# awslabs/dgl-ke

Measured on NVIDIA H100. Metric: edges/sec TransE_l2 d=400 neg=200 at 1/2/4/8 H100 vs ref CPU; HBM GB/s %peak, higher is better.
Workload: dtype f32

## Files before the change

### dgl-ke_b200/csrc/kge_rows.cu

```cuda
#include "kge_common.cuh"

namespace kge {


constexpr int kRowBlock = 256;
constexpr int kWarpsPerBlock = kRowBlock / kWarp;

__global__ void __launch_bounds__(kRowBlock) k_gather(TableView t, const long long* __restrict__ idx,
                                                       long long n, float* __restrict__ out) {
  long long job = (long long)blockIdx.x * kWarpsPerBlock + (threadIdx.x >> 5);
  if (job >= n) return;
  int lane = threadIdx.x & 31;
  const float* src = row_ptr(t, idx[job]);
  float* dst = out + job * (long long)t.dim;
  int nv = t.dim >> 2;
  for (int v = lane; v < nv; v += kWarp) st4(dst + 4 * v, ld4_stream(src + 4 * v));
  for (int k = (nv << 2) + lane; k < t.dim; k += kWarp) dst[k] = src[k];
}

void launch_gather(const LaunchCtx& c, const TableView& t, const long long* idx, long long n, float* out) {
  if (n <= 0) return;
  KGE_LAUNCH(c, k_gather, ceil_div(n, kWarpsPerBlock), kRowBlock, 0, t, idx, n, out);
}

// ... 458 lines not shown
  if (lane == 0) {
    float ps = pos[i];
    float wb = wt ? *wbar : 1.f;
    if (p.pairwise) {
      pl[i] = 0.f;
      gpos[i] = gp;
    } else {
      float dd;
      pl[i] = crit(r, ps, 1.f, dd);
      gpos[i] = dd * wb * r.inv2B;
    }
    nl[i] = nls;
    if (r.l2) rowsum[i] = rs;
  }
}

__global__ void __launch_bounds__(256) k_colsum(StepParams p, const float* __restrict__ V, float* __restrict__ colsum) {
  __shared__ float part[8][33];
  const int c = blockIdx.y, j = blockIdx.x * 32 + (threadIdx.x & 31), w = threadIdx.x >> 5;
  float s = 0.f;
  if (j < p.Ns) {
    const float* v = V + ((long long)c * p.Cs) * p.Ns + j;
    for (int i = w; i < p.Cs; i += 8) s += v[(long long)i * p.Ns];
  }
  part[w][threadIdx.x & 31] = s;
  __syncthreads();
  if (w == 0 && j < p.Ns) {
    float t = 0.f;
#pragma unroll
    for (int q = 0; q < 8; ++q) t += part[q][threadIdx.x];
    colsum[(long long)c * p.Ns + j] = t;
  }
}

__device__ __forceinline__ float block_sum(float v, float* sh) {
  v = warp_sum(v);
  int w = threadIdx.x >> 5, l = threadIdx.x & 31;
  __syncthreads();
  if (l == 0) sh[w] = v;
  __syncthreads();
  float r = (threadIdx.x < (blockDim.x >> 5)) ? sh[threadIdx.x] : 0.f;
  if (w == 0) r = warp_sum(r);
  return r;
}

__global__ void __launch_bounds__(1024) k_mean(const float* __restrict__ x, long long n, float* __restrict__ out) {
  __shared__ float sh[32];
  float s = 0.f;
  for (long long i = threadIdx.x; i < n; i += blockDim.x) s += x[i];
  s = block_sum(s, sh);
  if (threadIdx.x == 0) *out = s / (float)n;
}

constexpr int kRedBlocks = 64;
__device__ void reduce_log_part(const StepParams& p, const StepWs& w, long long nreg, const float* wbar, float* log4,
                                int bid, int nb) {
  __shared__ float sh[32];
  __shared__ bool last;
  const float *pl = w.pl, *nl = w.nl, *regp = w.regp;
  float* partial = w.red_partial;
  unsigned int* ticket = w.red_ticket;
  float a = 0.f, b = 0.f, r = 0.f;
  const long long t0 = (long long)bid * blockDim.x + threadIdx.x, stride = (long long)nb * blockDim.x;
  for (long long i = t0; i < p.B; i += stride) { a += pl[i]; b += nl[i]; }
  for (long long i = t0; i < nreg; i += stride) r += regp[i];
  a = block_sum(a, sh);
  b = block_sum(b, sh);
  r = block_sum(r, sh);
  if (threadIdx.x == 0) {
    partial[bid * 3 + 0] = a; partial[bid * 3 + 1] = b; partial[bid * 3 + 2] = r;
    __threadfence();
    unsigned int t = atomicAdd(ticket, 1u);
    last = (t == (unsigned int)nb - 1);
  }
  __syncthreads();
  if (last) {
    __threadfence();
    float sa = 0.f, sb = 0.f, sr = 0.f;
    if ((int)threadIdx.x < nb) {
      sa = ((volatile float*)partial)[threadIdx.x * 3 + 0];
      sb = ((volatile float*)partial)[threadIdx.x * 3 + 1];
      sr = ((volatile float*)partial)[threadIdx.x * 3 + 2];
    }
    sa = block_sum(sa, sh);
    sb = block_sum(sb, sh);
    sr = block_sum(sr, sh);
    if (threadIdx.x == 0) {
      float pos_loss = sa / (float)p.B * (wbar ? *wbar : 1.f);
      float neg_loss = sb / (float)p.B;
      log4[0] = p.pairwise ? 0.f : pos_loss; log4[1] = p.pairwise ? 0.f : neg_loss;
      log4[2] = p.pairwise ? neg_loss : (neg_loss + pos_loss) / 2.f;
      log4[3] = p.reg_coef * sr;
      *ticket = 0u;
    }
  }
}

__global__ void __launch_bounds__(256) k_reduce_log(StepParams p, StepWs w, long long nreg, const float* __restrict__ wbar,
                                                     float* __restrict__ log4) {
  if (nreg > 0 && p.U_dev) nreg = p.B + p.Nn + *p.U_dev;
  reduce_log_part(p, w, nreg, wbar, log4, blockIdx.x, gridDim.x);
}

void launch_wbar(const LaunchCtx& c, const StepParams& p, const float* wt, const StepWs& w) {
  if (wt) KGE_LAUNCH(c, k_mean, 1, 1024, 0, wt, p.B, w.wbar);
}

void launch_reduce_log(const LaunchCtx& c, const StepParams& p, const float* wt, const StepWs& w, float* log4,
                       bool want_reg) {
  const bool reg_on = want_reg && (p.reg_coef > 0.f && p.reg_norm > 0);
  if (log4)
    KGE_LAUNCH(c, k_reduce_log, kRedBlocks, 256, 0, p, w, reg_on ? (p.B + p.Nn + p.U) : 0, wt ? w.wbar : nullptr, log4);
}

void launch_loss_rows(const LaunchCtx& c, const StepParams& p, const float* pos, const float* S, const float* wt,
                      const StepWs& w) {
  KGE_LAUNCH(c, k_loss, ceil_div(p.B, kWarpsPerBlock), kRowBlock, 0, p, pos, S, wt, w.wbar, w.V, w.gpos, w.rowsum,
             w.pl, w.nl, w.Vhi, w.Vlo, w.VhiT, w.VloT);
}

void launch_colsum(const LaunchCtx& c, const StepParams& p, const StepWs& w) {
  if (p.model == KGE_TRANSE_L2) KGE_LAUNCH(c, k_colsum, dim3(ceil_div(p.Ns, 32), p.C), 256, 0, p, w.V, w.colsum);
}

void launch_loss(const LaunchCtx& c, const StepParams& p, const float* pos, const float* S, const float* wt,
                 const StepWs& w, float* log4, bool want_reg) {
  launch_wbar(c, p, wt, w);
  launch_loss_rows(c, p, pos, S, wt, w);
  launch_colsum(c, p, w);
  launch_reduce_log(c, p, wt, w, log4, want_reg);
}

template <int MODEL, int KIT>
__global__ void __launch_bounds__(kRowBlock) k_chain(StepParams p, TableView ent, TableView rel, BatchView b, StepWs w) {
  const long long i = (long long)blockIdx.x * kWarpsPerBlock + (threadIdx.x >> 5);
  if (i >= p.B) return;
  const int lane = threadIdx.x & 31;
  const long long hl = b.head_local[i], tl = b.tail_local[i], rid = b.rel_ids[i];
  const float* h = head_row(p, ent, b, w, i);
  const float* t = tail_row(p, ent, b, w, i);
  const float* r = row_ptr(rel, rid);
  const float* ga = w.GA + i * (long long)p.D;
  float* ngh = w.NG + hl * (long long)p.D;
  float* ngt = w.NG + tl * (long long)p.D;
  float* gr = p.rel_dense ? (w.rg + rid * (long long)p.Dr) : (w.GR + i * (long long)p.Dr);
  const bool dense = p.rel_dense != 0;
  auto rel_out = [&](int col, float4 v) { if (dense) red_add4(gr + col, v); else st4(gr + col, v); };
  const float gp = w.gpos[i];
  float gs = 0.f;

  if (MODEL == KGE_COMPLEX || MODEL == KGE_ROTATE) {
    const int half = p.D >> 1, nvh = half >> 2;
    const float den = p.emb_init / 3.14159265358979323846f;
    for (int v = lane; v < nvh; v += kWarp) {
      float4 hr = ld4(h + 4 * v), hi = ld4(h + half + 4 * v);
      float4 tr = ld4(t + 4 * v), ti = ld4(t + half + 4 * v);
      float4 gre = ld4(ga + 4 * v), gim = ld4(ga + half + 4 * v);
      float4 cr, ci, ph;
      if (MODEL == KGE_COMPLEX) { cr = ld4(r + 4 * v); ci = ld4(r + half + 4 * v); }
      else { ph = ld4(r + 4 * v); phase_cos_sin(ph, den, cr, ci); }
      float4 dhr, dhi, dtr, dti, dcr, dci;
      if (MODEL == KGE_COMPLEX) {
        dhr = f4_scale(f4_add(f4_mul(tr, cr), f4_mul(ti, ci)), gp);
        dhi = f4_scale(f4_sub(f4_mul(ti, cr), f4_mul(tr, ci)), gp);
        dtr = f4_scale(f4_sub(f4_mul(hr, cr), f4_mul(hi, ci)), gp);
        dti = f4_scale(f4_add(f4_mul(hi, cr), f4_mul(hr, ci)), gp);
        dcr = f4_scale(f4_add(f4_mul(hr, tr), f4_mul(hi, ti)), gp);
        dci = f4_scale(f4_sub(f4_mul(hr, ti), f4_mul(hi, tr)), gp);
      } else {
        float4 dre = f4_sub(f4_sub(f4_mul(hr, cr), f4_mul(hi, ci)), tr);
        float4 dim = f4_sub(f4_add(f4_mul(hr, ci), f4_mul(hi, cr)), ti);
        float4 qre, qim;
#define KGE_Q(c_)                                                                    \
        { float m = sqrtf(dre.c_ * dre.c_ + dim.c_ * dim.c_); float s_ = (m > 0.f) ? (-gp / m) : 0.f; \
          qre.c_ = dre.c_ * s_; qim.c_ = dim.c_ * s_; }
        KGE_Q(x) KGE_Q(y) KGE_Q(z) KGE_Q(w)
#undef KGE_Q
        dhr = f4_add(f4_mul(qre, cr), f4_mul(qim, ci));
        dhi = f4_sub(f4_mul(qim, cr), f4_mul(qre, ci));
        dtr = f4_neg(qre);
        dti = f4_neg(qim);
        dcr = f4_add(f4_mul(qre, hr), f4_mul(qim, hi));
        dci = f4_sub(f4_mul(qim, hr), f4_mul(qre, hi));
      }
      if (p.neg_head) {
        dtr = f4_add(dtr, f4_sub(f4_mul(gre, cr), f4_mul(gim, ci)));
        dti = f4_add(dti, f4_add(f4_mul(gre, ci), f4_mul(gim, cr)));
        dcr = f4_add(dcr, f4_add(f4_mul(gre, tr), f4_mul(gim, ti)));
        dci = f4_add(dci, f4_sub(f4_mul(gre, ti), f4_mul(gim, tr)));
      } else {
        dhr = f4_add(dhr, f4_add(f4_mul(gre, cr), f4_mul(gim, ci)));
        dhi = f4_add(dhi, f4_sub(f4_mul(gim, cr), f4_mul(gre, ci)));
        dcr = f4_add(dcr, f4_add(f4_mul(gre, hr), f4_mul(gim, hi)));
        dci = f4_add(dci, f4_sub(f4_mul(gim, hr), f4_mul(gre, hi)));
      }
      red_add4(ngh + 4 * v, dhr); red_add4(ngh + half + 4 * v, dhi);
      red_add4(ngt + 4 * v, dtr); red_add4(ngt + half + 4 * v, dti);
      if (MODEL == KGE_COMPLEX) {
        float4 g0 = f4_add(dcr, reg_grad4(cr, p.reg_norm, p.reg_coef));
        float4 g1 = f4_add(dci, reg_grad4(ci, p.reg_norm, p.reg_coef));
        rel_out(4 * v, g0); rel_out(half + 4 * v, g1);
        gs += f4_dot(g0, g0) + f4_dot(g1, g1);
      } else {
        float4 dth = f4_sub(f4_mul(dci, cr), f4_mul(dcr, ci));
        float4 g0 = make_float4(dth.x / den, dth.y / den, dth.z / den, dth.w / den);
        g0 = f4_add(g0, reg_grad4(ph, p.reg_norm, p.reg_coef));
        rel_out(4 * v, g0);
        gs += f4_dot(g0, g0);
      }
    }
  } else {
    const int nv = p.D >> 2;
    float nrm_scale = 0.f, rsum = 0.f;
    if (MODEL == KGE_TRANSE_L2) {
      float n = w.pnorm[i];
      nrm_scale = (n > 0.f) ? (-gp / n) : 0.f;
      rsum = w.rowsum[i];
    }
    const float4 z4 = make_float4(0.f, 0.f, 0.f, 0.f);
    for (int v0 = 0; v0 < nv; v0 += kWarp * KIT) {
      float4 hq[KIT], rq[KIT], tq[KIT], gq[KIT];
#pragma unroll
      for (int it = 0; it < KIT; ++it) {
        const int v = v0 + lane + kWarp * it;
        const bool ok = v < nv;
        hq[it] = ok ? ld4(h + 4 * v) : z4; rq[it] = ok ? ld4(r + 4 * v) : z4;
        tq[it] = ok ? ld4(t + 4 * v) : z4; gq[it] = ok ? ld4(ga + 4 * v) : z4;
      }
#pragma unroll
      for (int it = 0; it < KIT; ++it) {
        const int v = v0 + lane + kWarp * it;
        if (v >= nv) continue;
        const float4 h4 = hq[it], r4 = rq[it], t4 = tq[it], g4 = gq[it];
        float4 dh, dt, dr;
        if (MODEL == KGE_TRANSE_L1 || MODEL == KGE_TRANSE_L2) {
          float4 e = f4_sub(f4_add(h4, r4), t4);
          float4 u;
          if (MODEL == KGE_TRANSE_L2) u = f4_scale(e, nrm_scale);
          else u = make_float4(-gp * sgnf(e.x), -gp * sgnf(e.y), -gp * sgnf(e.z), -gp * sgnf(e.w));
          float4 a = p.neg_head ? f4_sub(t4, r4) : f4_add(h4, r4);
          float4 gA = (MODEL == KGE_TRANSE_L2) ? f4_fma(a, -rsum, g4) : g4;
          if (p.neg_head) { dt = f4_sub(gA, u); dr = f4_sub(u, gA); dh = u; }
          else            { dh = f4_add(u, gA); dr = dh; dt = f4_neg(u); }
        } else {
          dh = f4_scale(f4_mul(r4, t4), gp);
          dr = f4_scale(f4_mul(h4, t4), gp);
          dt = f4_scale(f4_mul(h4, r4), gp);
          if (p.neg_head) { dt = f4_add(dt, f4_mul(g4, r4)); dr = f4_add(dr, f4_mul(g4, t4)); }
          else            { dh = f4_add(dh, f4_mul(g4, r4)); dr = f4_add(dr, f4_mul(g4, h4)); }
        }
        red_add4(ngh + 4 * v, dh);
        red_add4(ngt + 4 * v, dt);
        dr = f4_add(dr, reg_grad4(r4, p.reg_norm, p.reg_coef));
        rel_out(4 * v, dr);
        gs += f4_dot(dr, dr);
      }
    }
  }
  gs = warp_sum(gs);
  if (lane == 0) {
    if (dense) atomicAdd(w.rgs + rid, gs / (float)p.Dr);
    else w.gsr[i] = gs / (float)p.Dr;
  }
}

void launch_chain(const LaunchCtx& c, const StepParams& p, const TableView& ent, const TableView& rel,
                  const BatchView& b, const StepWs& w) {
  if (ent.n_shards > 1) {
    KGE_DISPATCH_MODEL(p.model, KGE_LAUNCH(c, (k_chain<M, 4>), ceil_div(p.B, kWarpsPerBlock), kRowBlock, 0, p, ent, rel, b, w));
  } else {
    KGE_DISPATCH_MODEL(p.model, KGE_LAUNCH(c, (k_chain<M, 1>), ceil_div(p.B, kWarpsPerBlock), kRowBlock, 0, p, ent, rel, b, w));
  }
}

struct UpdArgs {
  StepParams p;
  TableView ent, rel;
  BatchView b;
  StepWs w;
  float* log4;
  const float* wt;
  int phase_lo, phase_hi;
  int bulk_red;
};

__device__ __forceinline__ unsigned int ld_acquire_u32(const unsigned int* p) {
  unsigned int v;
  asm volatile("ld.acquire.gpu.global.u32 %0, [%1];" : "=r"(v) : "l"(p) : "memory");
  return v;
}
__device__ __forceinline__ void grid_barrier(unsigned int* ctr) {
  __syncthreads();
  if (threadIdx.x == 0) {
    __threadfence();
    atomicAdd(ctr, 1u);
    while (ld_acquire_u32(ctr) < gridDim.x) __nanosleep(200);
    __threadfence();
  }
  __syncthreads();
}

constexpr int kRedRowFloats = 512;
struct RedStage {
  float* buf[2];
  unsigned n;
};
__device__ __forceinline__ float* red_stage_acquire(RedStage& r, int lane) {
  if (lane == 0) asm volatile("cp.async.bulk.wait_group.read 1;" ::: "memory");
  __syncwarp();
  return r.buf[r.n & 1u];
}
__device__ __forceinline__ void red_stage_issue(RedStage& r, float* dst, int dim, int lane) {
  asm volatile("fence.proxy.async.shared::cta;" ::: "memory");
  __syncwarp();
  if (lane == 0) {
    asm volatile("cp.reduce.async.bulk.global.shared::cta.bulk_group.add.f32 [%0], [%1], %2;"
                 :: "l"(dst), "r"((unsigned)__cvta_generic_to_shared(r.buf[r.n & 1u])), "r"((unsigned)dim * 4u) : "memory");
    asm volatile("cp.async.bulk.commit_group;" ::: "memory");
  }
  ++r.n;
}
__device__ __forceinline__ void red_stage_drain(int lane) {
  if (lane == 0) asm volatile("cp.async.bulk.wait_group 0;" ::: "memory");
  __syncwarp();
}
__device__ __forceinline__ void st_shared4(float* p, float4 v) { *reinterpret_cast<float4*>(p) = v; }

__device__ __forceinline__ void upd_node(const StepParams& p, const TableView& ent, const BatchView& b, const StepWs& w,
                                         long long u, int lane, RedStage* rs) {
  const long long id = b.node_ids[u];
  float* row = row_ptr(ent, id);
  float* ng = w.NG + u * (long long)p.D;
  const float* nc = node_row(p, ent, b, w, u);
  const int nv = p.D >> 2;
  const float4 z = make_float4(0.f, 0.f, 0.f, 0.f);
  const bool sharded = ent.n_shards > 1;
  const bool reg_on = (p.reg_coef > 0.f && p.reg_norm > 0);
  float* st = state_ptr(ent, id);
  if (nv <= 4 * kWarp) {
    float4 x[4], gq[4];
#pragma unroll
    for (int q = 0; q < 4; ++q) {
      const int v = lane + kWarp * q;
      x[q] = (v < nv) ? ld4(nc + 4 * v) : z;
      gq[q] = (v < nv) ? ld4(ng + 4 * v) : z;
    }
    float gs = 0.f, reg = 0.f;
#pragma unroll
    for (int q = 0; q < 4; ++q) {
      gq[q] = f4_add(gq[q], reg_grad4(x[q], p.reg_norm, p.reg_coef));
      gs += f4_dot(gq[q], gq[q]);
      if (reg_on && node_reg_in_update(p)) reg += abs_pow4_sum(x[q], p.reg_norm);
    }
    gs = warp_sum(gs) / (float)p.D;
    if (node_reg_in_update(p)) {
      reg = warp_sum(reg);
      if (lane == 0) w.regp[p.B + p.Nn + u] = reg;
    }
    float* st = state_ptr(ent, id);
    float s_new = 0.f;
    if (lane == 0) {
      if (sharded) s_new = atomicAdd_system(st, gs) + gs;
      else { s_new = *st + gs; *st = s_new; }
    }
    s_new = __shfl_sync(0xffffffffu, s_new, 0);
    const float nlr_std = -p.lr / (sqrtf(s_new) + 1e-10f);
    float* stage = (sharded && rs) ? red_stage_acquire(*rs, lane) : nullptr;
#pragma unroll
    for (int q = 0; q < 4; ++q) {
      const int v = lane + kWarp * q;
      if (v < nv) {
        if (stage) st_shared4(stage + 4 * v, f4_scale(gq[q], nlr_std));
        else if (sharded) red_add4_sys(row + 4 * v, f4_scale(gq[q], nlr_std));
        else st4(row + 4 * v, f4_fma(gq[q], nlr_std, x[q]));
        st4(ng + 4 * v, z);
      }
    }
    if (stage) red_stage_issue(*rs, row, p.D, lane);
    return;
  }
  float gs = 0.f, reg = 0.f;
  for (int v = lane; v < nv; v += kWarp) {
    const float4 x = ld4(nc + 4 * v);
    float4 g = f4_add(ld4(ng + 4 * v), reg_grad4(x, p.reg_norm, p.reg_coef));
    gs += f4_dot(g, g);
    if (reg_on && node_reg_in_update(p)) reg += abs_pow4_sum(x, p.reg_norm);
  }
  gs = warp_sum(gs) / (float)p.D;
  if (node_reg_in_update(p)) {
    reg = warp_sum(reg);
    if (lane == 0) w.regp[p.B + p.Nn + u] = reg;
  }
  float s_new = 0.f;
  if (lane == 0) {
    if (sharded) s_new = atomicAdd_system(st, gs) + gs;
    else { s_new = *st + gs; *st = s_new; }
  }
  s_new = __shfl_sync(0xffffffffu, s_new, 0);
  const float stdv = sqrtf(s_new) + 1e-10f;
  const float nlr_std = -p.lr / stdv;
  for (int v = lane; v < nv; v += kWarp) {
    float4 x = ld4(nc + 4 * v);
    float4 g = f4_add(ld4(ng + 4 * v), reg_grad4(x, p.reg_norm, p.reg_coef));
    const float4 tmp = f4_scale(g, nlr_std);
    if (sharded) red_add4_sys(row + 4 * v, tmp);
    else st4(row + 4 * v, f4_add(x, tmp));
    st4(ng + 4 * v, z);
  }
}

__device__ __forceinline__ void upd_rel_dense(const TableView& rel, float* rg, float* rgs, long long r, float lr, int lane) {
  const float gs = rgs[r];
  if (gs == 0.f) return;
  float* st = state_ptr(rel, r);
  float s_new = 0.f;
  if (lane == 0) { s_new = *st + gs; *st = s_new; }
  s_new = __shfl_sync(0xffffffffu, s_new, 0);
  __syncwarp();
  if (lane == 0) rgs[r] = 0.f;
  const float stdv = sqrtf(s_new) + 1e-10f;
  float* row = row_ptr(rel, r);
  float* g = rg + r * (long long)rel.dim;
  const float4 z = make_float4(0.f, 0.f, 0.f, 0.f);
  for (int v = lane; v < (rel.dim >> 2); v += kWarp) {
    float4 x = ld4(g + 4 * v), e = ld4(row + 4 * v);
    st4(row + 4 * v, f4_fma(x, -lr / stdv, e));
    st4(g + 4 * v, z);
  }
}

__device__ __forceinline__ void apply_row(const TableView& t, long long id, const float* g, int dim, float lr, int lane,
                                          RedStage* rs = nullptr) {
  float* row = row_ptr(t, id);
  const int nv = dim >> 2;
  if (nv <= 4 * kWarp && (dim & 3) == 0) {
    float4 x[4];
#pragma unroll
    for (int q = 0; q < 4; ++q) {
      const int v = lane + kWarp * q;
      x[q] = (v < nv) ? ld4(g + 4 * v) : make_float4(0.f, 0.f, 0.f, 0.f);
    }
    const float nlr_std = -lr / (sqrtf(*state_ptr(t, id)) + 1e-10f);
    if (rs) {
      float* stage = red_stage_acquire(*rs, lane);
#pragma unroll
      for (int q = 0; q < 4; ++q) {
        const int v = lane + kWarp * q;
        if (v < nv) st_shared4(stage + 4 * v, f4_scale(x[q], nlr_std));
      }
      red_stage_issue(*rs, row, dim, lane);
      return;
    }
#pragma unroll
    for (int q = 0; q < 4; ++q) {
      const int v = lane + kWarp * q;
      if (v < nv) table_red_add4(t, row + 4 * v, f4_scale(x[q], nlr_std));
    }
    return;
  }
  const float stdv = sqrtf(*state_ptr(t, id)) + 1e-10f;
  const float nlr_std = -lr / stdv;
  for (int v = lane; v < nv; v += kWarp) {
    float4 x = ld4(g + 4 * v);
    table_red_add4(t, row + 4 * v, f4_scale(x, nlr_std));
  }
  for (int k = (nv << 2) + lane; k < dim; k += kWarp) atomicAdd(row + k, (-lr * g[k]) / stdv);
}

__device__ void reduce_log_part(const StepParams& p, const StepWs& w, long long nreg, const float* wbar, float* log4,
                                int bid, int nb);

__global__ void __launch_bounds__(kRowBlock, 4) k_update(UpdArgs a) {
  __shared__ __align__(128) float red_stage[kWarpsPerBlock][2][kRedRowFloats];
  const StepParams& p = a.p;
  const StepWs& w = a.w;
  const int lane = threadIdx.x & 31;
  RedStage rstage{{red_stage[threadIdx.x >> 5][0], red_stage[threadIdx.x >> 5][1]}, 0u};
  RedStage* rs = a.bulk_red ? &rstage : nullptr;
  const long long warp0 = (long long)blockIdx.x * kWarpsPerBlock + (threadIdx.x >> 5);
  const long long nwarps = (long long)gridDim.x * kWarpsPerBlock;
  const bool rel_edge = !p.rel_deferred && !p.rel_dense;
  for (int phase = a.phase_lo; phase <= a.phase_hi; ++phase) {
    if (phase == 1) {
      const long long nrel = (p.rel_dense && !p.rel_deferred) ? a.rel.num_rows : 0;
      const long long U = node_count(p);
      for (long long j = warp0; j < U + nrel; j += nwarps) {
        if (j < U) upd_node(p, a.ent, a.b, w, j, lane, rs);
        else upd_rel_dense(a.rel, w.rg, w.rgs, j - U, p.lr, lane);
      }
    } else if (phase == 2) {
      if (p.fused) {
        const long long t0 = (long long)blockIdx.x * blockDim.x + threadIdx.x, nt = (long long)gridDim.x * blockDim.x;
        for (long long j = t0; j < p.Nn; j += nt) table_atomic_add(a.ent, state_ptr(a.ent, a.b.neg_ids[j]), w.gsn[j]);
      } else {
        for (long long j = warp0; j < p.Nn; j += nwarps) {
          const float* g = w.Bn + j * (long long)p.D;
          float gs = 0.f;
          for (int v = lane; v < (p.D >> 2); v += kWarp) { float4 x = ld4(g + 4 * v); gs += f4_dot(x, x); }
          gs = warp_sum(gs);
          if (lane == 0) table_atomic_add(a.ent, state_ptr(a.ent, a.b.neg_ids[j]), gs / (float)p.D);
        }
      }
      if (rel_edge) {
        const long long t0 = (long long)blockIdx.x * blockDim.x + threadIdx.x, nt = (long long)gridDim.x * blockDim.x;
        for (long long i = t0; i < p.B; i += nt) table_atomic_add(a.rel, state_ptr(a.rel, a.b.rel_ids[i]), w.gsr[i]);
      }
    } else {
      const long long nr = rel_edge ? p.B : 0;
      for (long long j = warp0; j < p.Nn + nr; j += nwarps) {
        if (j < p.Nn) apply_row(a.ent, a.b.neg_ids[j], w.Bn + j * (long long)p.D, p.D, p.lr, lane, rs);
        else apply_row(a.rel, a.b.rel_ids[j - p.Nn], w.GR + (j - p.Nn) * (long long)p.Dr, p.Dr, p.lr, lane);
      }
      if (a.log4) {
        const int nb = gridDim.x < 64 ? gridDim.x : 64;
        const bool reg_on = (p.reg_coef > 0.f && p.reg_norm > 0);
        if ((int)blockIdx.x < nb)
          reduce_log_part(p, w, reg_on ? (p.B + p.Nn + node_count(p)) : 0, a.wt ? w.wbar : nullptr, a.log4, blockIdx.x, nb);
      }
    }
    if (phase < a.phase_hi) grid_barrier(w.sync_ctr + (phase - 1));
  }
  if (rs) red_stage_drain(lane);
  if (a.phase_hi > a.phase_lo) {
    __syncthreads();
    if (threadIdx.x == 0) {
      __threadfence();
      if (atomicAdd(w.sync_ctr + 3, 1u) == gridDim.x - 1) {
        w.sync_ctr[0] = 0u; w.sync_ctr[1] = 0u; w.sync_ctr[2] = 0u;
        __threadfence();
        w.sync_ctr[3] = 0u;
      }
    }
  }
}

int launch_update(const LaunchCtx& c, const StepParams& p, const TableView& ent, const TableView& rel,
                  const BatchView& b, const StepWs& w, float* log4, const float* wt) {
  static const bool no_bulk = getenv("KGE_B200_NO_BULKRED") != nullptr;
  UpdArgs a{p, ent, rel, b, w, log4, wt, 1, 3, (!no_bulk && p.D <= kRedRowFloats && (p.D & 3) == 0) ? 1 : 0};
  const long long nrel = (p.rel_dense && !p.rel_deferred) ? rel.num_rows : 0;
  const long long nr = (!p.rel_deferred && !p.rel_dense) ? p.B : 0;
  long long jobs = p.U + nrel;
  if (p.Nn + nr > jobs) jobs = p.Nn + nr;
  static int occ[64] = {};
  int dev = 0;
  cudaGetDevice(&dev);
  if (dev >= 0 && dev < 64 && occ[dev] == 0) {
    int n = 0;
    if (cudaOccupancyMaxActiveBlocksPerMultiprocessor(&n, k_update, kRowBlock, 0) != cudaSuccess || n < 1) n = 1;
    occ[dev] = n;
  }
  static const bool no_coop = getenv("KGE_B200_NO_COOP") != nullptr;
  const int sms = (p.rel_deferred && c.num_sms > 32) ? c.num_sms - 16 : c.num_sms;
  const int max_resident = sms * (dev >= 0 && dev < 64 ? occ[dev] : 1);
  int grid = ceil_div(jobs, kWarpsPerBlock);
  if (!no_coop) {
    if (grid > max_resident) grid = max_resident;
    void* args[] = {&a};
    prof_begin(c, "k_update<nodes | state adds | apply>");
    cudaError_t e = cudaLaunchCooperativeKernel((void*)k_update, dim3(grid), dim3(kRowBlock), args, 0, c.stream);
    prof_end(c);
    if (c.launch_counter) ++*c.launch_counter;
    if (e == cudaSuccess) return KGE_OK;
    cudaGetLastError();
    return fail(KGE_ERR_CUDA, "cooperative launch of k_update failed: %s (set KGE_B200_NO_COOP=1 for the three-launch form)",
                cudaGetErrorString(e));
  }
  for (int ph = 1; ph <= 3; ++ph) {
    a.phase_lo = a.phase_hi = ph;
    const char* nm = ph == 1 ? "k_update<nodes>" : (ph == 2 ? "k_update<state adds>" : "k_update<apply>");
    KGE_LAUNCH_NAMED(c, nm, k_update, grid, kRowBlock, 0, a);
  }
  return KGE_OK;
}

__global__ void __launch_bounds__(kRowBlock) k_state_add(TableView t, const long long* __restrict__ idx,
                                                          const float* __restrict__ grad, long long n, int dim) {
  const long long j = (long long)blockIdx.x * kWarpsPerBlock + (threadIdx.x >> 5);
  if (j >= n) return;
  const int lane = threadIdx.x & 31;
  const float* g = grad + j * (long long)dim;
  float gs = 0.f;
  for (int v = lane; v < (dim >> 2); v += kWarp) { float4 x = ld4(g + 4 * v); gs += f4_dot(x, x); }
  for (int k = ((dim >> 2) << 2) + lane; k < dim; k += kWarp) gs += g[k] * g[k];
  gs = warp_sum(gs);
  if (lane == 0) table_atomic_add(t, state_ptr(t, idx[j]), gs / (float)dim);
}
__global__ void __launch_bounds__(kRowBlock) k_apply(TableView t, const long long* __restrict__ idx,
                                                      const float* __restrict__ grad, long long n, int dim, float lr) {
  const long long j = (long long)blockIdx.x * kWarpsPerBlock + (threadIdx.x >> 5);
  if (j >= n) return;
  apply_row(t, idx[j], grad + j * (long long)dim, dim, lr, threadIdx.x & 31);
}

__global__ void __launch_bounds__(kRowBlock) k_rel_accumulate(StepParams p, BatchView b, StepWs w,
                                                               float* __restrict__ rg, float* __restrict__ rgs) {
  const long long i = (long long)blockIdx.x * kWarpsPerBlock + (threadIdx.x >> 5);
  if (i >= p.B) return;
  const int lane = threadIdx.x & 31;
  const long long rid = b.rel_ids[i];
  const float* g = w.GR + i * (long long)p.Dr;
  float* dst = rg + rid * (long long)p.Dr;
  for (int v = lane; v < (p.Dr >> 2); v += kWarp) red_add4(dst + 4 * v, ld4(g + 4 * v));
  if (lane == 0) atomicAdd(rgs + rid, w.gsr[i]);
}

__global__ void __launch_bounds__(kRowBlock) k_rel_apply_dense(TableView rel, float* __restrict__ rg,
                                                                float* __restrict__ rgs, float lr) {
  const long long r = (long long)blockIdx.x * kWarpsPerBlock + (threadIdx.x >> 5);
  if (r >= rel.num_rows) return;
  const int lane = threadIdx.x & 31;
  const float gs = rgs[r];
  if (gs == 0.f) return;
  float* st = state_ptr(rel, r);
  float s_new = 0.f;
  if (lane == 0) { s_new = *st + gs; *st = s_new; rgs[r] = 0.f; }
  s_new = __shfl_sync(0xffffffffu, s_new, 0);
  const float stdv = sqrtf(s_new) + 1e-10f;
  float* row = row_ptr(rel, r);
  float* g = rg + r * (long long)rel.dim;
  const float4 z = make_float4(0.f, 0.f, 0.f, 0.f);
  for (int v = lane; v < (rel.dim >> 2); v += kWarp) {
    float4 x = ld4(g + 4 * v), e = ld4(row + 4 * v);
    st4(row + 4 * v, f4_fma(x, -lr / stdv, e));
    st4(g + 4 * v, z);
  }
}

void launch_rel_grad_dense(const LaunchCtx& c, const StepParams& p, const BatchView& b, const StepWs& w, float* rg,
                           float* rgs) {
  KGE_LAUNCH(c, k_rel_accumulate, ceil_div(p.B, kWarpsPerBlock), kRowBlock, 0, p, b, w, rg, rgs);
}
void launch_rel_apply_dense(const LaunchCtx& c, const TableView& rel, float* rg, float* rgs, float lr) {
  KGE_LAUNCH(c, k_rel_apply_dense, ceil_div(rel.num_rows, kWarpsPerBlock), kRowBlock, 0, rel, rg, rgs, lr);
}

void launch_adagrad(const LaunchCtx& c, const TableView& t, const long long* idx, const float* grad, long long n,
                    float lr) {
  if (n <= 0) return;
  KGE_LAUNCH(c, k_state_add, ceil_div(n, kWarpsPerBlock), kRowBlock, 0, t, idx, grad, n, t.dim);
  KGE_LAUNCH(c, k_apply, ceil_div(n, kWarpsPerBlock), kRowBlock, 0, t, idx, grad, n, t.dim, lr);
}

__global__ void __launch_bounds__(kRowBlock) k_node_grad_reg(StepParams p, TableView ent, BatchView b, StepWs w,
                                                              float* __restrict__ out) {
  const long long u = (long long)blockIdx.x * kWarpsPerBlock + (threadIdx.x >> 5);
  if (u >= node_count(p)) return;
  const int lane = threadIdx.x & 31;
  const float* row = node_row(p, ent, b, w, u);
  for (int v = lane; v < (p.D >> 2); v += kWarp)
    st4(out + u * (long long)p.D + 4 * v,
        f4_add(ld4(w.NG + u * (long long)p.D + 4 * v), reg_grad4(ld4(row + 4 * v), p.reg_norm, p.reg_coef)));
}
void launch_node_grad_with_reg(const LaunchCtx& c, const StepParams& p, const TableView& ent, const BatchView& b,
                               const StepWs& w, float* out) {
  KGE_LAUNCH(c, k_node_grad_reg, ceil_div(p.U, kWarpsPerBlock), kRowBlock, 0, p, ent, b, w, out);
}

}
```

Before: 33.23 million.

## Restructure update kernel phases with index prefetch and early state loads

New measurement: 35.14 million, median of 6. 5.7% higher.

```diff
diff --git a/dgl-ke_b200/csrc/kge_rows.cu b/dgl-ke_b200/csrc/kge_rows.cu
--- a/dgl-ke_b200/csrc/kge_rows.cu
+++ b/dgl-ke_b200/csrc/kge_rows.cu
@@ -784,20 +784,21 @@
 
 constexpr int kRedRowFloats = 512;
 struct RedStage {
-  float* buf[2];
+  float* buf;
   unsigned n;
 };
+__device__ __forceinline__ float* red_stage_buf(const RedStage& r) { return r.buf + (r.n & 1u) * kRedRowFloats; }
 __device__ __forceinline__ float* red_stage_acquire(RedStage& r, int lane) {
   if (lane == 0) asm volatile("cp.async.bulk.wait_group.read 1;" ::: "memory");
   __syncwarp();
-  return r.buf[r.n & 1u];
+  return red_stage_buf(r);
 }
 __device__ __forceinline__ void red_stage_issue(RedStage& r, float* dst, int dim, int lane) {
   asm volatile("fence.proxy.async.shared::cta;" ::: "memory");
   __syncwarp();
   if (lane == 0) {
     asm volatile("cp.reduce.async.bulk.global.shared::cta.bulk_group.add.f32 [%0], [%1], %2;"
-                 :: "l"(dst), "r"((unsigned)__cvta_generic_to_shared(r.buf[r.n & 1u])), "r"((unsigned)dim * 4u) : "memory");
+                 :: "l"(dst), "r"((unsigned)__cvta_generic_to_shared(red_stage_buf(r))), "r"((unsigned)dim * 4u) : "memory");
     asm volatile("cp.async.bulk.commit_group;" ::: "memory");
   }
   ++r.n;
@@ -808,17 +809,26 @@
 }
 __device__ __forceinline__ void st_shared4(float* p, float4 v) { *reinterpret_cast<float4*>(p) = v; }
 
+__device__ __forceinline__ float upd_state(float* st, float st_old, float gs, bool sharded, int lane) {
+  float s_new = 0.f;
+  if (lane == 0) {
+    if (sharded) s_new = atomicAdd_system(st, gs) + gs;
+    else { s_new = st_old + gs; *st = s_new; }
+  }
+  return __shfl_sync(0xffffffffu, s_new, 0);
+}
+
 __device__ __forceinline__ void upd_node(const StepParams& p, const TableView& ent, const BatchView& b, const StepWs& w,
-                                         long long u, int lane, RedStage* rs) {
-  const long long id = b.node_ids[u];
+                                         long long u, long long id, int lane, RedStage& rs) {
   float* row = row_ptr(ent, id);
   float* ng = w.NG + u * (long long)p.D;
-  const float* nc = node_row(p, ent, b, w, u);
+  const float* nc = p.use_nc ? (w.NC + u * (long long)p.D) : row;
   const int nv = p.D >> 2;
   const float4 z = make_float4(0.f, 0.f, 0.f, 0.f);
   const bool sharded = ent.n_shards > 1;
   const bool reg_on = (p.reg_coef > 0.f && p.reg_norm > 0);
   float* st = state_ptr(ent, id);
+  const float st_old = (!sharded && lane == 0) ? *st : 0.f;
   if (nv <= 4 * kWarp) {
     float4 x[4], gq[4];
 #pragma unroll
@@ -839,15 +849,9 @@
       reg = warp_sum(reg);
       if (lane == 0) w.regp[p.B + p.Nn + u] = reg;
     }
-    float* st = state_ptr(ent, id);
-    float s_new = 0.f;
-    if (lane == 0) {
-      if (sharded) s_new = atomicAdd_system(st, gs) + gs;
-      else { s_new = *st + gs; *st = s_new; }
-    }
-    s_new = __shfl_sync(0xffffffffu, s_new, 0);
+    const float s_new = upd_state(st, st_old, gs, sharded, lane);
     const float nlr_std = -p.lr / (sqrtf(s_new) + 1e-10f);
-    float* stage = (sharded && rs) ? red_stage_acquire(*rs, lane) : nullptr;
+    float* stage = (sharded && rs.buf) ? red_stage_acquire(rs, lane) : nullptr;
 #pragma unroll
     for (int q = 0; q < 4; ++q) {
       const int v = lane + kWarp * q;
@@ -858,7 +862,7 @@
         st4(ng + 4 * v, z);
       }
     }
-    if (stage) red_stage_issue(*rs, row, p.D, lane);
+    if (stage) red_stage_issue(rs, row, p.D, lane);
     return;
   }
   float gs = 0.f, reg = 0.f;
@@ -873,12 +877,7 @@
     reg = warp_sum(reg);
     if (lane == 0) w.regp[p.B + p.Nn + u] = reg;
   }
-  float s_new = 0.f;
-  if (lane == 0) {
-    if (sharded) s_new = atomicAdd_system(st, gs) + gs;
-    else { s_new = *st + gs; *st = s_new; }
-  }
-  s_new = __shfl_sync(0xffffffffu, s_new, 0);
+  const float s_new = upd_state(st, st_old, gs, sharded, lane);
   const float stdv = sqrtf(s_new) + 1e-10f;
   const float nlr_std = -p.lr / stdv;
   for (int v = lane; v < nv; v += kWarp) {
@@ -891,20 +890,43 @@
   }
 }
 
-__device__ __forceinline__ void upd_rel_dense(const TableView& rel, float* rg, float* rgs, long long r, float lr, int lane) {
-  const float gs = rgs[r];
-  if (gs == 0.f) return;
-  float* st = state_ptr(rel, r);
+__device__ __forceinline__ float upd_rel_state(float* st, float st_old, float gs, float* gs_src, int lane) {
   float s_new = 0.f;
-  if (lane == 0) { s_new = *st + gs; *st = s_new; }
+  if (lane == 0) { s_new = st_old + gs; *st = s_new; }
   s_new = __shfl_sync(0xffffffffu, s_new, 0);
   __syncwarp();
-  if (lane == 0) rgs[r] = 0.f;
-  const float stdv = sqrtf(s_new) + 1e-10f;
+  if (lane == 0) *gs_src = 0.f;
+  return s_new;
+}
+__device__ __forceinline__ void upd_rel_dense(const TableView& rel, float* rg, float* rgs, long long r, float lr, int lane) {
+  float* st = state_ptr(rel, r);
   float* row = row_ptr(rel, r);
   float* g = rg + r * (long long)rel.dim;
+  const int nv = rel.dim >> 2;
   const float4 z = make_float4(0.f, 0.f, 0.f, 0.f);
-  for (int v = lane; v < (rel.dim >> 2); v += kWarp) {
+  const float gs = rgs[r], st_old = (lane == 0) ? *st : 0.f;
+  if (nv <= 4 * kWarp) {
+    float4 x[4], e[4];
+#pragma unroll
+    for (int q = 0; q < 4; ++q) {
+      const int v = lane + kWarp * q;
+      x[q] = (v < nv) ? ld4(g + 4 * v) : z;
+      e[q] = (v < nv) ? ld4(row + 4 * v) : z;
+    }
+    if (gs == 0.f) return;
+    const float s_new = upd_rel_state(st, st_old, gs, rgs + r, lane);
+    const float stdv = sqrtf(s_new) + 1e-10f;
+#pragma unroll
+    for (int q = 0; q < 4; ++q) {
+      const int v = lane + kWarp * q;
+      if (v < nv) { st4(row + 4 * v, f4_fma(x[q], -lr / stdv, e[q])); st4(g + 4 * v, z); }
+    }
+    return;
+  }
+  if (gs == 0.f) return;
+  const float s_new = upd_rel_state(st, st_old, gs, rgs + r, lane);
+  const float stdv = sqrtf(s_new) + 1e-10f;
+  for (int v = lane; v < nv; v += kWarp) {
     float4 x = ld4(g + 4 * v), e = ld4(row + 4 * v);
     st4(row + 4 * v, f4_fma(x, -lr / stdv, e));
     st4(g + 4 * v, z);
@@ -912,7 +934,7 @@
 }
 
 __device__ __forceinline__ void apply_row(const TableView& t, long long id, const float* g, int dim, float lr, int lane,
-                                          RedStage* rs = nullptr) {
+                                          RedStage& rs) {
   float* row = row_ptr(t, id);
   const int nv = dim >> 2;
   if (nv <= 4 * kWarp && (dim & 3) == 0) {
@@ -923,14 +945,14 @@
       x[q] = (v < nv) ? ld4(g + 4 * v) : make_float4(0.f, 0.f, 0.f, 0.f);
     }
     const float nlr_std = -lr / (sqrtf(*state_ptr(t, id)) + 1e-10f);
-    if (rs) {
-      float* stage = red_stage_acquire(*rs, lane);
+    if (rs.buf) {
+      float* stage = red_stage_acquire(rs, lane);
 #pragma unroll
       for (int q = 0; q < 4; ++q) {
         const int v = lane + kWarp * q;
         if (v < nv) st_shared4(stage + 4 * v, f4_scale(x[q], nlr_std));
       }
-      red_stage_issue(*rs, row, dim, lane);
+      red_stage_issue(rs, row, dim, lane);
       return;
     }
 #pragma unroll
@@ -952,57 +974,66 @@
 __device__ void reduce_log_part(const StepParams& p, const StepWs& w, long long nreg, const float* wbar, float* log4,
                                 int bid, int nb);
 
-__global__ void __launch_bounds__(kRowBlock, 4) k_update(UpdArgs a) {
+__global__ void __launch_bounds__(kRowBlock, 2) k_update(UpdArgs a) {
   __shared__ __align__(128) float red_stage[kWarpsPerBlock][2][kRedRowFloats];
   const StepParams& p = a.p;
   const StepWs& w = a.w;
   const int lane = threadIdx.x & 31;
-  RedStage rstage{{red_stage[threadIdx.x >> 5][0], red_stage[threadIdx.x >> 5][1]}, 0u};
-  RedStage* rs = a.bulk_red ? &rstage : nullptr;
-  const long long warp0 = (long long)blockIdx.x * kWarpsPerBlock + (threadIdx.x >> 5);
-  const long long nwarps = (long long)gridDim.x * kWarpsPerBlock;
+  RedStage rs{a.bulk_red ? red_stage[threadIdx.x >> 5][0] : nullptr, 0u};
+  RedStage per_lane{nullptr, 0u};
+  const int warp0 = (int)blockIdx.x * kWarpsPerBlock + (int)(threadIdx.x >> 5);
+  const int nwarps = (int)gridDim.x * kWarpsPerBlock;
   const bool rel_edge = !p.rel_deferred && !p.rel_dense;
-  for (int phase = a.phase_lo; phase <= a.phase_hi; ++phase) {
-    if (phase == 1) {
-      const long long nrel = (p.rel_dense && !p.rel_deferred) ? a.rel.num_rows : 0;
-      const long long U = node_count(p);
-      for (long long j = warp0; j < U + nrel; j += nwarps) {
-        if (j < U) upd_node(p, a.ent, a.b, w, j, lane, rs);
-        else upd_rel_dense(a.rel, w.rg, w.rgs, j - U, p.lr, lane);
-      }
-    } else if (phase == 2) {
-      if (p.fused) {
-        const long long t0 = (long long)blockIdx.x * blockDim.x + threadIdx.x, nt = (long long)gridDim.x * blockDim.x;
-        for (long long j = t0; j < p.Nn; j += nt) table_atomic_add(a.ent, state_ptr(a.ent, a.b.neg_ids[j]), w.gsn[j]);
-      } else {
-        for (long long j = warp0; j < p.Nn; j += nwarps) {
-          const float* g = w.Bn + j * (long long)p.D;
-          float gs = 0.f;
-          for (int v = lane; v < (p.D >> 2); v += kWarp) { float4 x = ld4(g + 4 * v); gs += f4_dot(x, x); }
-          gs = warp_sum(gs);
-          if (lane == 0) table_atomic_add(a.ent, state_ptr(a.ent, a.b.neg_ids[j]), gs / (float)p.D);
-        }
-      }
-      if (rel_edge) {
-        const long long t0 = (long long)blockIdx.x * blockDim.x + threadIdx.x, nt = (long long)gridDim.x * blockDim.x;
-        for (long long i = t0; i < p.B; i += nt) table_atomic_add(a.rel, state_ptr(a.rel, a.b.rel_ids[i]), w.gsr[i]);
-      }
+  if (a.phase_lo <= 1) {
+    const long long nrel = (p.rel_dense && !p.rel_deferred) ? a.rel.num_rows : 0;
+    const long long U = node_count(p);
+    long long id = (warp0 < U) ? a.b.node_ids[warp0] : 0;
+    for (long long j = warp0; j < U + nrel; j += nwarps) {
+      const long long cur = id;
+      if (j + nwarps < U) id = a.b.node_ids[j + nwarps];
+      if (j < U) upd_node(p, a.ent, a.b, w, j, cur, lane, rs);
+      else upd_rel_dense(a.rel, w.rg, w.rgs, j - U, p.lr, lane);
+    }
+    if (a.phase_hi > 1) grid_barrier(w.sync_ctr + 0);
+  }
+  if (a.phase_lo <= 2 && a.phase_hi >= 2) {
+    if (p.fused) {
+      const long long t0 = (long long)blockIdx.x * blockDim.x + threadIdx.x, nt = (long long)gridDim.x * blockDim.x;
+      for (long long j = t0; j < p.Nn; j += nt) table_atomic_add(a.ent, state_ptr(a.ent, a.b.neg_ids[j]), w.gsn[j]);
     } else {
-      const long long nr = rel_edge ? p.B : 0;
-      for (long long j = warp0; j < p.Nn + nr; j += nwarps) {
-        if (j < p.Nn) apply_row(a.ent, a.b.neg_ids[j], w.Bn + j * (long long)p.D, p.D, p.lr, lane, rs);
-        else apply_row(a.rel, a.b.rel_ids[j - p.Nn], w.GR + (j - p.Nn) * (long long)p.Dr, p.Dr, p.lr, lane);
-      }
-      if (a.log4) {
-        const int nb = gridDim.x < 64 ? gridDim.x : 64;
-        const bool reg_on = (p.reg_coef > 0.f && p.reg_norm > 0);
-        if ((int)blockIdx.x < nb)
-          reduce_log_part(p, w, reg_on ? (p.B + p.Nn + node_count(p)) : 0, a.wt ? w.wbar : nullptr, a.log4, blockIdx.x, nb);
-      }
-    }
-    if (phase < a.phase_hi) grid_barrier(w.sync_ctr + (phase - 1));
-  }
-  if (rs) red_stage_drain(lane);
+      for (long long j = warp0; j < p.Nn; j += nwarps) {
+        const float* g = w.Bn + j * (long long)p.D;
+        float gs = 0.f;
+        for (int v = lane; v < (p.D >> 2); v += kWarp) { float4 x = ld4(g + 4 * v); gs += f4_dot(x, x); }
+        gs = warp_sum(gs);
+        if (lane == 0) table_atomic_add(a.ent, state_ptr(a.ent, a.b.neg_ids[j]), gs / (float)p.D);
+      }
+    }
+    if (rel_edge) {
+      const long long t0 = (long long)blockIdx.x * blockDim.x + threadIdx.x, nt = (long long)gridDim.x * blockDim.x;
+      for (long long i = t0; i < p.B; i += nt) table_atomic_add(a.rel, state_ptr(a.rel, a.b.rel_ids[i]), w.gsr[i]);
+    }
+    if (a.phase_hi > 2) grid_barrier(w.sync_ctr + 1);
+  }
+  if (a.phase_hi >= 3) {
+    const long long nr = rel_edge ? p.B : 0;
+    auto job_id = [&](long long j) { return j < p.Nn ? a.b.neg_ids[j] : (j < p.Nn + nr ? a.b.rel_ids[j - p.Nn] : 0); };
+    long long id = job_id(warp0);
+    for (long long j = warp0; j < p.Nn + nr; j += nwarps) {
+      const long long cur = id;
+      id = job_id(j + nwarps);
+      if (j < p.Nn) apply_row(a.ent, cur, w.Bn + j * (long long)p.D, p.D, p.lr, lane, rs);
+      else apply_row(a.rel, cur, w.GR + (j - p.Nn) * (long long)p.Dr, p.Dr, p.lr, lane, per_lane);
+    }
+    if (a.log4) {
+      const int nb = gridDim.x < 64 ? gridDim.x : 64;
+      const int bid = (int)blockIdx.x - ((int)gridDim.x - nb);
+      const bool reg_on = (p.reg_coef > 0.f && p.reg_norm > 0);
+      if (bid >= 0)
+        reduce_log_part(p, w, reg_on ? (p.B + p.Nn + node_count(p)) : 0, a.wt ? w.wbar : nullptr, a.log4, bid, nb);
+    }
+  }
+  if (rs.buf) red_stage_drain(lane);
   if (a.phase_hi > a.phase_lo) {
     __syncthreads();
     if (threadIdx.x == 0) {
@@ -1072,7 +1103,8 @@
                                                       const float* __restrict__ grad, long long n, int dim, float lr) {
   const long long j = (long long)blockIdx.x * kWarpsPerBlock + (threadIdx.x >> 5);
   if (j >= n) return;
-  apply_row(t, idx[j], grad + j * (long long)dim, dim, lr, threadIdx.x & 31);
+  RedStage per_lane{nullptr, 0u};
+  apply_row(t, idx[j], grad + j * (long long)dim, dim, lr, threadIdx.x & 31, per_lane);
 }
 
 __global__ void __launch_bounds__(kRowBlock) k_rel_accumulate(StepParams p, BatchView b, StepWs w,
```
